# LuoGroup2023/PanTax

Measured on AMD Instinct MI355X. Metric: PAO wall-time (s) + Mreads/s: packed reads + DB (graphs and their unique-trio index) resident in HBM -> abundance tables; the metric's own GAF -> abundance quantity is value_gaf_to_tables (files -> tables, never `value`), higher is better.
Workload: dtype int64+f64

## Files before the change

pantax_amd/csrc/api_step.cpp:

```cpp
#include <algorithm>
#include <cmath>
#include <chrono>
#include <cstdio>
#include <cstdlib>
#include <cstring>
#include <vector>
#include "lad.hpp"

using namespace ptx;

namespace {
struct SpOut { Db *db; uint8_t *keep; double *absolute; int slot; };
void copy_species_out(void *arg) {
    SpOut *o = static_cast<SpOut *>(arg);
    const uint32_t S = o->db->S;
    std::memcpy(o->absolute, o->db->h_sp_out[o->slot].p, sizeof(double) * S);
    std::memcpy(o->keep, o->db->h_sp_out[o->slot].p + sizeof(double) * S, S);
}

int step_enqueue(pantax_hip_ctx *ctx, pantax_hip_db *db, pantax_hip_reads *reads, const double *avg_len, const pantax_hip_step_config *cfg) {
    if (db->d_node_rec.p == nullptr) return fail(ctx, PANTAX_HIP_E_STATE, "profile_step: the db was uploaded without graphs (ranges only)");
    if (db->step_inflight >= 2) return fail(ctx, PANTAX_HIP_E_STATE, "profile_step_enqueue: two steps of this db are already in flight; collect one first");
    const uint32_t S = db->S;
    const int slot = db->step_enq;
    const auto t_begin = std::chrono::steady_clock::now();
    double marks[8] = {0}; int n_marks = 0;
    auto mark = [&]() { if (n_marks < 8) marks[n_marks++] = std::chrono::duration<double, std::milli>(std::chrono::steady_clock::now() - t_begin).count(); };
    struct SlowReport { double *m; int *n; bool on; ~SlowReport() {
        if (*n && m[*n - 1] > 2.0 && on) {
            std::fprintf(stderr, "[step_enqueue] slow call, ms at marks (trio enqueued, bin+species, prezero+cov prepare, coverage, strain):");
            for (int i = 0; i < *n; ++i) std::fprintf(stderr, " %.2f", m[i]);
            std::fprintf(stderr, "\n");
        } } } slow_report{marks, &n_marks, ctx->cfg.trace};
    bool forked = false;
    if (cfg->rebuild_trio && !(db->trio_prefetched && db->trio_built)) { db->trio_built = false; db->cov_done = false; db->U = 0; }
    db->trio_prefetched = false;
    if (!db->trio_built) {
        if (db->trio_free_valid && !ctx->cfg.trio_after_step) PTX_HIP(ctx, hipStreamWaitEvent(ctx->stream2, db->ev_trio_free, 0));
        else {
            PTX_HIP(ctx, hipEventRecord(ctx->ev_seq, ctx->stream));
            PTX_HIP(ctx, hipStreamWaitEvent(ctx->stream2, ctx->ev_seq, 0));
        }
        hipStream_t main_stream = ctx->stream;
        ctx->stream_main = main_stream; ctx->stream = ctx->stream2;
        const int rc = trio_index_build(ctx, db, false);
        const hipError_t e = hipEventRecord(ctx->ev_fork, ctx->stream2);
        ctx->stream = main_stream; ctx->stream_main = nullptr;
        if (rc != 0) return rc;
        PTX_HIP(ctx, e);
        forked = true;
    }
    struct ForkGuard {
        Ctx *c; Db *d; bool armed;
        ~ForkGuard() { if (armed) { (void)hipStreamSynchronize(c->stream2); d->trio_built = false; d->cov_done = false; } }
    } fork_guard{ctx, db, forked};
// ... 98 lines not shown
```

pantax_amd/csrc/common.hpp:

```cpp
#pragma once
#include <hip/hip_runtime.h>
#include <cstdint>
#include <cstdio>
#include <map>
#include <functional>
#include <mutex>
#include <cstring>
#include <atomic>
#include <string>
#include <vector>
#include "../../include/pantax_hip.h"

#ifndef TRIO_LH_PACK
#define TRIO_LH_PACK 0
#endif
namespace ptx {

struct Ctx;
#if TRIO_LH_PACK
using trio_len_t = uint2;
#else
using trio_len_t = uint32_t;
#endif

// ... 86 lines not shown
    int stage_ch_mb = 0;
    bool stream_prio = true;
    int dev_cache_gb = -1;
    bool numa_bind = true;
    uint64_t gaf_piece_bytes = 0;
    int db_groups = 0;
    uint64_t db_path_steps_max = 0;
    std::string trio_path;
    std::string trio_rows;
    int uniq_hash = -1;
    std::string mask;
    std::string row_sort;
    std::string objective;
    std::string read_strain_route, evidence_route, depth_route, near_miss_route, hap_pairs_route;
    int hap_pairs_chunk = 0;
    int depth_grid = 0;
    int near_miss_words = 0;
    bool cov_general = false;
    std::string cov_long;
    int covl_shape = -1;
    bool cov_count = false;
    int cov_clean_async = -1;
    bool cov_self_clean = false;
    bool walk_sum_in_bin = false;
    int ncs_prefix_min = 48;
    bool ncs_no_prefix = false;
    bool cov_arena_verify = false;
    int cov_item_groups = 0;
    int tv_u = 4, tv_rounds = 4, tf_u = 8, tf_rounds = 1, rows_u = 1, tb_slots = 256, trio_xcd = 3, cov_shape = -1, covf_shape = -1, cov_xcd = 0, group_bucket_bits = 0;
    uint32_t tv_ablate = 0, cov_ablate = 0, ssn_ablate = 0;
    bool trio_two_pass = false;
    std::string bin_route;
    std::string node_pass;
    std::string lad_shape;
    std::string scan_tile;
    std::string ssn_keys;
    bool ssn_poison_keys = false;
    int ssn_ties_async = -1;
    bool no_absent_skip = false;
    bool ssn_debug = false, scan_no_huge = false, flag_rank_chained = false, ratio_kernel = false, mask_pass = false, trio_free_at_filter = false,
         trio_after_step = false;
};
int ctx_set_option(CtxConfig &cfg, const char *name, const char *value);

struct NumaInfo {
    int node = -1;
    std::vector<int> cpus;
};

struct Ctx {
    std::recursive_mutex mu;
    CtxConfig cfg;
    NumaInfo numa;
    int device = 0;
    hipStream_t stream = nullptr;
    hipStream_t stream_main = nullptr;
    hipStream_t stream2 = nullptr;
    hipStream_t stream_up = nullptr;
    hipEvent_t ev_fork = nullptr;
    hipEvent_t ev_ssn_fork = nullptr, ev_ssn_join = nullptr;
    hipEvent_t ev_seq = nullptr;
    std::string err;
    std::mutex err_mu;
    bool timing = false;
    std::string timing_filter;
    std::vector<TimedLaunch> pending;
// ... 423 lines not shown
```

pantax_amd/csrc/ctx.cpp:

```cpp
#include <exception>
#include <cstdarg>
#include <algorithm>
#include <atomic>
#include <cstring>
#include <functional>
#include <chrono>
#include <condition_variable>
#include <cstdio>
#include <mutex>
#include <thread>
#include <unistd.h>
#include <fcntl.h>
#include <sched.h>
#include <pthread.h>
#include <sys/syscall.h>
#include <fstream>
#include <cctype>
#include <cstddef>
#include <cstdlib>
#include "common.hpp"
#include "lad.hpp"

namespace ptx {

// ... 39 lines not shown
KTimer::~KTimer() {
    if (!start) return;
    (void)hipEventRecord(stop, ctx->stream);
    ctx->pending.push_back({name, start, stop});
}

int collect_timings(Ctx *ctx) {
    if (ctx->pending.empty()) return 0;
    PTX_HIP(ctx, hipStreamSynchronize(ctx->stream));
    for (auto &t : ctx->pending) {
        float ms = 0.f;
        if (hipEventElapsedTime(&ms, t.start, t.stop) == hipSuccess) {
            auto &a = ctx->acc[t.name];
            a.first += 1;
            a.second += ms;
        }
        ctx->free_events.push_back({t.start, t.stop});
    }
    ctx->pending.clear();
    return 0;
}

namespace {
enum OptKind { O_BOOL, O_INT, O_U32, O_U64, O_STR };
struct OptDesc { const char *name; OptKind kind; size_t off; };
#define OPT(nm, kind, field) {nm, kind, offsetof(CtxConfig, field)}
const OptDesc OPTIONS[] = {
    OPT("hip_trace", O_BOOL, trace), OPT("stage_threads", O_INT, stage_threads), OPT("stage_ch_mb", O_INT, stage_ch_mb), OPT("stream_prio", O_BOOL, stream_prio), OPT("numa_bind", O_BOOL, numa_bind), OPT("dev_cache_gb", O_INT, dev_cache_gb),
    OPT("gaf_piece_bytes", O_U64, gaf_piece_bytes), OPT("db_path_steps_max", O_U64, db_path_steps_max), OPT("db_groups", O_INT, db_groups), OPT("trio_path", O_STR, trio_path), OPT("trio_rows", O_STR, trio_rows), OPT("trio_two_pass", O_BOOL, trio_two_pass), OPT("uniq_hash", O_INT, uniq_hash),
    OPT("mask", O_STR, mask), OPT("row_sort", O_STR, row_sort), OPT("objective", O_STR, objective), OPT("read_strain_route", O_STR, read_strain_route), OPT("evidence_route", O_STR, evidence_route), OPT("depth_route", O_STR, depth_route), OPT("depth_grid", O_INT, depth_grid), OPT("near_miss_route", O_STR, near_miss_route), OPT("near_miss_words", O_INT, near_miss_words), OPT("hap_pairs_route", O_STR, hap_pairs_route), OPT("hap_pairs_chunk", O_INT, hap_pairs_chunk),
    OPT("cov_general", O_BOOL, cov_general), OPT("cov_long", O_STR, cov_long), OPT("covl_shape", O_INT, covl_shape), OPT("cov_count", O_BOOL, cov_count), OPT("cov_self_clean", O_BOOL, cov_self_clean), OPT("cov_clean_async", O_INT, cov_clean_async), OPT("cov_arena_verify", O_BOOL, cov_arena_verify), OPT("ncs_no_prefix", O_BOOL, ncs_no_prefix), OPT("ncs_prefix_min", O_INT, ncs_prefix_min), OPT("walk_sum_in_bin", O_BOOL, walk_sum_in_bin), OPT("cov_item_groups", O_INT, cov_item_groups), OPT("tv_u", O_INT, tv_u), OPT("tv_rounds", O_INT, tv_rounds), OPT("tf_u", O_INT, tf_u), OPT("tf_rounds", O_INT, tf_rounds),
    OPT("rows_u", O_INT, rows_u), OPT("tb_slots", O_INT, tb_slots), OPT("trio_xcd", O_INT, trio_xcd), OPT("cov_shape", O_INT, cov_shape),
    OPT("covf_shape", O_INT, covf_shape), OPT("cov_xcd", O_INT, cov_xcd), OPT("group_bucket_bits", O_INT, group_bucket_bits), OPT("tv_ablate", O_U32, tv_ablate),
    OPT("cov_ablate", O_U32, cov_ablate), OPT("ssn_ablate", O_U32, ssn_ablate), OPT("no_absent_skip", O_BOOL, no_absent_skip), OPT("node_pass", O_STR, node_pass), OPT("bin_route", O_STR, bin_route), OPT("lad_shape", O_STR, lad_shape), OPT("ssn_debug", O_BOOL, ssn_debug),
    OPT("ssn_keys", O_STR, ssn_keys), OPT("ssn_poison_keys", O_BOOL, ssn_poison_keys), OPT("ssn_ties_async", O_INT, ssn_ties_async),
    OPT("scan_no_huge", O_BOOL, scan_no_huge), OPT("scan_tile", O_STR, scan_tile), OPT("flag_rank_chained", O_BOOL, flag_rank_chained), OPT("ratio_kernel", O_BOOL, ratio_kernel),
    OPT("mask_pass", O_BOOL, mask_pass), OPT("trio_free_at_filter", O_BOOL, trio_free_at_filter), OPT("trio_after_step", O_BOOL, trio_after_step),
};
#undef OPT
}

int ctx_set_option(CtxConfig &cfg, const char *name, const char *value) {
    if (!name) return PANTAX_HIP_E_INVALID;
    static const CtxConfig defaults;
    for (const OptDesc &o : OPTIONS) {
        if (std::strcmp(o.name, name) != 0) continue;
        char *dst = reinterpret_cast<char *>(&cfg) + o.off;
        const char *def = reinterpret_cast<const char *>(&defaults) + o.off;
        char *end = nullptr;
        switch (o.kind) {
        case O_BOOL: *reinterpret_cast<bool *>(dst) = value ? !(value[0] == '0' || value[0] == '\0' || value[0] == 'n' || value[0] == 'f') : *reinterpret_cast<const bool *>(def); return 0;
        case O_INT: { if (!value) { *reinterpret_cast<int *>(dst) = *reinterpret_cast<const int *>(def); return 0; }
                      const long v = std::strtol(value, &end, 10); if (end == value) return PANTAX_HIP_E_INVALID; *reinterpret_cast<int *>(dst) = (int)v; return 0; }
        case O_U32: { if (!value) { *reinterpret_cast<uint32_t *>(dst) = *reinterpret_cast<const uint32_t *>(def); return 0; }
                      const unsigned long long v = std::strtoull(value, &end, 10); if (end == value) return PANTAX_HIP_E_INVALID; *reinterpret_cast<uint32_t *>(dst) = (uint32_t)v; return 0; }
        case O_U64: { if (!value) { *reinterpret_cast<uint64_t *>(dst) = *reinterpret_cast<const uint64_t *>(def); return 0; }
                      const unsigned long long v = std::strtoull(value, &end, 10); if (end == value) return PANTAX_HIP_E_INVALID; *reinterpret_cast<uint64_t *>(dst) = (uint64_t)v; return 0; }
        case O_STR: *reinterpret_cast<std::string *>(dst) = value ? value : ""; return 0;
        }
    }
    return PANTAX_HIP_E_INVALID;
}

static void config_from_env(CtxConfig &cfg) {
    for (const OptDesc &o : OPTIONS) {
        std::string env = "PANTAX_";
        for (const char *p = o.name; *p; ++p) env += (char)std::toupper((unsigned char)*p);
// ... 591 lines not shown
```

pantax_amd/csrc/sample_sort_nodes.hip:

```cpp
#include <algorithm>
#include <cstdio>
#include <vector>
#include "ssn_device.hpp"

namespace ptx {

size_t sample_sort_nodes_ws_elems(uint32_t S, uint64_t seg_bound, uint64_t V) { return ssn_plan(S, seg_bound, V).total_words; }

int sample_sort_nodes(Ctx *ctx, const double *ab, const uint64_t *mask, const uint32_t *d_node_base, uint32_t S, uint64_t seg_bound, uint64_t V,
                      uint64_t *rows16, uint64_t *const k[3], int pack_shift, uint32_t *d_ws, uint32_t *d_n, const RowPatterns *pat,
                      const RowMaskSource *haps, const NodeCovSource *fused) {
    if (S == 0 || V == 0) {
        PTX_HIP(ctx, hipMemsetAsync(d_n, 0, sizeof(uint32_t), ctx->stream));
        if (pat) { PTX_HIP(ctx, hipMemsetAsync(pat->d_K, 0, sizeof(uint32_t), ctx->stream)); PTX_HIP(ctx, hipMemsetAsync(pat->sp_pat_off, 0, (S + 1) * sizeof(uint32_t), ctx->stream));
                   PTX_HIP(ctx, hipMemsetAsync(pat->pat_start, 0, sizeof(uint32_t), ctx->stream)); }
        return 0;
    }
    if (seg_bound > SSN_MAX_SEG) return fail(ctx, PANTAX_HIP_E_LIMIT, "sample_sort_nodes: a segment of %llu nodes exceeds %llu", (unsigned long long)seg_bound, (unsigned long long)SSN_MAX_SEG);
    if (S > 65535) return fail(ctx, PANTAX_HIP_E_LIMIT, "sample_sort_nodes: %u segments exceed the launch grid", S);
    if (haps) { if (haps->max_haps > 64) return fail(ctx, PANTAX_HIP_E_INVALID, "sample_sort_nodes: masks from haplotype words take species of at most 64 haplotypes"); }
    else if (!mask) return fail(ctx, PANTAX_HIP_E_INVALID, "sample_sort_nodes: neither a mask array nor haplotype words");
    if (fused && (!haps || !fused->bases || !fused->bit_off || !fused->full || !fused->bitmap || !fused->amax || !fused->nvalid || !fused->nzsum || !fused->nzcnt))
        return fail(ctx, PANTAX_HIP_E_INVALID, "sample_sort_nodes: the fused node pass takes haplotype words and the coverage arena");
    if (!fused && !ab) return fail(ctx, PANTAX_HIP_E_INVALID, "sample_sort_nodes: no abundance array");

    const int keys_all = ssn_keys_all(ctx->cfg.ssn_keys.c_str(), pat != nullptr);
    if (keys_all < 0) return fail(ctx, PANTAX_HIP_E_INVALID, "sample_sort_nodes: option ssn_keys=%s%s", ctx->cfg.ssn_keys.c_str(), pat ? "" : " (a sort whose caller reads the keys stores all of them)");

    const SsnPlan pl = ssn_plan(S, seg_bound, V);
    Sn sn;
    sn.node_base = d_node_base; sn.ab = ab; sn.mask = haps ? nullptr : mask;
    if (haps) sn.hp = *haps;
    if (fused) { sn.fz = *fused; sn.ab = nullptr; sn.hp.cov = nullptr; }
    sn.G = pl.G; sn.per = pl.per;
    sn.ablate = ctx->cfg.ssn_ablate;
    sn.skip_empty = ctx->cfg.no_absent_skip ? 0u : 1u;
    sn.ws = d_ws + pl.ws;
    sn.cntm = d_ws + pl.cntm;
    sn.stage_cnt = d_ws + pl.stage_cnt;
    sn.c0p = reinterpret_cast<double *>(d_ws + pl.c0p);
    sn.c0 = pat ? pat->c0 : nullptr;
    sn.seg_n = d_ws + pl.seg_n; sn.seg_out = d_ws + pl.seg_out;
    uint32_t *sub_k = d_ws + pl.sub_k;
    sn.ids = reinterpret_cast<uint16_t *>(d_ws + pl.ids);
    sn.npart = reinterpret_cast<NodePartial *>(d_ws + pl.npart);
    sn.rows = reinterpret_cast<ulonglong2 *>(rows16);
    sn.stage = reinterpret_cast<ulonglong2 *>(rows16) + V;
    sn.ksp = pack_shift >= 0 ? nullptr : k[0];
    sn.km = pack_shift >= 0 ? k[0] : k[1];
    sn.ka = pack_shift >= 0 ? k[1] : k[2];
    sn.pack_shift = pack_shift;
    sn.keys_all = (uint32_t)keys_all;
    if (!keys_all && ctx->cfg.ssn_poison_keys) {
        PTX_TRY(byte_fill(ctx, sn.km, 0xA5, V * sizeof(uint64_t)));
        if (sn.ksp) PTX_TRY(byte_fill(ctx, sn.ksp, 0xA5, V * sizeof(uint64_t)));
    }

    { KTimer t(ctx, "ssn_sample_kernel");
      ssn_sample_launch(ctx, sn, S, fused != nullptr); }
    if (fused) {
        KTimer t(ctx, "node_rows_kernel");
        ssn_node_rows_launch(ctx, sn, S, haps->max_haps);
    } else {
        KTimer t(ctx, "ssn_hist_kernel");
        ssn_hist_launch(ctx, sn, S, haps != nullptr, haps ? haps->max_haps : 0u);
    }
    { KTimer t(ctx, "ssn_offsets_kernel");
      ssn_offsets_launch(ctx, sn, S, d_n); }
    const bool clocked = ctx->timing && ctx->timing_filter.empty();
    const bool ties_async = ssn_ties_async(ctx->cfg.ssn_ties_async, clocked, ctx->stream_main != nullptr, ctx->stream2 != nullptr);
    struct TieJoin {
        Ctx *c; bool armed;
        ~TieJoin() { if (armed) (void)hipStreamSynchronize(c->stream2); }
    } tie_join{ctx, false};
    if (ties_async) {
        if (!ctx->ev_ssn_fork) PTX_HIP(ctx, hipEventCreateWithFlags(&ctx->ev_ssn_fork, hipEventDisableTiming));
        if (!ctx->ev_ssn_join) PTX_HIP(ctx, hipEventCreateWithFlags(&ctx->ev_ssn_join, hipEventDisableTiming));
        PTX_HIP(ctx, hipEventRecord(ctx->ev_ssn_fork, ctx->stream));
        PTX_HIP(ctx, hipStreamWaitEvent(ctx->stream2, ctx->ev_ssn_fork, 0));
        hipStream_t main_stream = ctx->stream;
        ctx->stream_main = main_stream; ctx->stream = ctx->stream2;
        tie_join.armed = true;
        { KTimer t(ctx, "ssn_ties_kernel");
          ssn_ties_launch(ctx, sn, S, pl.tie_grid); }
        const hipError_t e = hipEventRecord(ctx->ev_ssn_join, ctx->stream2);
        ctx->stream = main_stream; ctx->stream_main = nullptr;
        PTX_HIP(ctx, e);
    }
    { KTimer t(ctx, "ssn_scatter_kernel");
      ssn_scatter_launch(ctx, sn, S); }
    if (!ties_async) {
        KTimer t(ctx, "ssn_ties_kernel");
        ssn_ties_launch(ctx, sn, S, pl.tie_grid);
    }
    { KTimer t(ctx, "ssn_local_wave_kernel");
// ... 38 lines not shown
```

pantax_amd/csrc/ssn_device.hpp:

```cpp
#pragma once
#include "primitives.hpp"
#include "wave.hpp"
#include "ssn_plan.hpp"

namespace ptx {

constexpr int SN_NSPLIT = SN_NLEAF - 1;
constexpr int SN_CAP = 4096;
constexpr int SN_WAVE_CAP = 512;
constexpr int SN_WAVE_CAP2 = 1024;
constexpr uint16_t SN_NO_ROW = 0xFFFFu;
static_assert(sizeof(NodePartial) == 4 * SN_NODE_PARTIAL_WORDS && alignof(NodePartial) == 8, "ssn_plan lays out [S x G] NodePartial at an even word offset");

struct Key2 { uint64_t m, a; };
__device__ __forceinline__ bool less2(const Key2 &x, const Key2 &y) { return (x.m < y.m) | ((x.m == y.m) & (x.a < y.a)); }
__device__ __forceinline__ bool eq2(const Key2 &x, const Key2 &y) { return (x.m == y.m) & (x.a == y.a); }

struct Sn {
    const uint32_t *node_base;
    const double *ab;
    const uint64_t *mask;
    RowMaskSource hp;
    NodeCovSource fz;
    NodePartial *npart;
// ... 92 lines not shown
__device__ __forceinline__ bool sn_pair_mixed(const ulonglong2 *__restrict__ tree, uint32_t j, uint64_t *mv = nullptr) {
    if (j == 0 || j >= (uint32_t)SN_NSPLIT) { if (mv) *mv = 0; return true; }
    const uint64_t ma = tree[tree_node(j - 1)].x, mb = tree[tree_node(j)].x;
    if (mv) *mv = mb;
    return ma != mb;
}

__device__ __forceinline__ void sn_tiles(const Sn &sn, uint32_t n, uint32_t g, uint32_t &t0, uint32_t &t1) {
    const uint32_t nt = (n + SN_TILE - 1) / SN_TILE;
    t0 = g * sn.per; t1 = t0 + sn.per;
    if (t0 > nt) t0 = nt;
    if (t1 > nt) t1 = nt;
}

template <int NT>
__device__ __forceinline__ void bitonic2(uint64_t *km, uint64_t *ka, uint32_t N) {
    for (uint32_t k = 2; k <= N; k <<= 1)
        for (uint32_t j = k >> 1; j > 0; j >>= 1) {
            for (uint32_t t = threadIdx.x; t < N / 2; t += NT) {
                const uint32_t i = ((t & ~(j - 1)) << 1) | (t & (j - 1)), l = i | j;
                const Key2 x{km[i], ka[i]}, y{km[l], ka[l]};
                const bool up = (i & k) == 0;
                if (up ? less2(y, x) : less2(x, y)) { km[i] = y.m; ka[i] = y.a; km[l] = x.m; ka[l] = x.a; }
            }
            __syncthreads();
        }
}

#ifdef SSN_ABLATE
#define SSN_ABL(b) ((sn.ablate & (b)) != 0u)
#else
#define SSN_ABL(b) false
#endif

void ssn_sample_launch(Ctx *ctx, const Sn &sn, uint32_t S, bool fused);
void ssn_node_rows_launch(Ctx *ctx, const Sn &sn, uint32_t S, uint32_t max_haps);
void ssn_hist_launch(Ctx *ctx, const Sn &sn, uint32_t S, bool haps, uint32_t max_haps);
void ssn_offsets_launch(Ctx *ctx, const Sn &sn, uint32_t S, uint32_t *d_n);
void ssn_scatter_launch(Ctx *ctx, const Sn &sn, uint32_t S);
void ssn_ties_launch(Ctx *ctx, const Sn &sn, uint32_t S, uint32_t tie_grid);
void ssn_local_launch(Ctx *ctx, const Sn &sn, uint32_t S);
void ssn_patterns_launch(Ctx *ctx, const Sn &sn, uint32_t S, uint32_t *sub_k, const RowPatterns &pat, const uint32_t *d_n);

}
```

pantax_amd/csrc/ssn_node_pass.hip:

```cpp
#include "ssn_device.hpp"

namespace ptx {

namespace {
template <bool HAPS>
__global__ void __launch_bounds__(256) ssn_hist_kernel(Sn sn) {
    __shared__ ulonglong2 tree[SN_NLEAF];
    __shared__ uint32_t s_hist[SN_NBUCKET];
    extern __shared__ unsigned long long s_dyn_tab[];
    __shared__ int s_bit[64];
    __shared__ unsigned long long s_acc[2 * 64];
    const uint32_t s = blockIdx.y, g = blockIdx.x, o = sn.node_base[s], n = sn.node_base[s + 1] - o;
    uint32_t *w = sn.w(s);
    if (n == 0 || w[SN_OFF_FLAGS] != 0) return;
    if (HAPS && sn.skip_empty && sn.hp.sp_p[s] <= 0) {
        uint32_t *row0 = sn.cntm + ((size_t)s * sn.G + g) * SN_NBUCKET;
        for (int i = threadIdx.x; i < SN_NBUCKET; i += 256) row0[i] = 0u;
        if (threadIdx.x == 0) { sn.stage_cnt[(size_t)s * sn.G + g] = 0u; if (sn.c0) sn.c0p[(size_t)s * sn.G + g] = 0.0; }
        return;
    }
    uint32_t t0, t1;
    sn_tiles(sn, n, g, t0, t1);
    const ulonglong2 *gt = reinterpret_cast<const ulonglong2 *>(w + SN_OFF_TREE);
    __shared__ uint32_t s_nstage;
// ... 92 lines not shown
                }
            }
        }
    }
    __syncthreads();
    uint32_t *row = sn.cntm + ((size_t)s * sn.G + g) * SN_NBUCKET;
    for (int i = threadIdx.x; i < SN_NBUCKET; i += 256) row[i] = s_hist[i];
    if (threadIdx.x == 0) sn.stage_cnt[(size_t)s * sn.G + g] = s_nstage;
    if (sn.c0) {
        __shared__ double s_c[4];
        cacc = wave_reduce(cacc, [](double x, double y) { return x + y; });
        if (lane == 0) s_c[threadIdx.x >> 6] = cacc;
        __syncthreads();
        if (threadIdx.x == 0) sn.c0p[(size_t)s * sn.G + g] = (s_c[0] + s_c[1]) + (s_c[2] + s_c[3]);
    }
    if (HAPS && p0 > 0 && sn.hp.ratio) {
#pragma unroll
        for (int k = 0; k < 8; ++k) {
            if (k >= p0) break;
            const unsigned long long cs = wave_reduce(c8[k], [](unsigned long long x, unsigned long long y) { return x + y; });
            const unsigned long long ls = wave_reduce(l8[k], [](unsigned long long x, unsigned long long y) { return x + y; });
            if (lane == 0) {
                if (cs) atomicAdd(&s_acc[2 * k], cs);
                if (ls) atomicAdd(&s_acc[2 * k + 1], ls);
            }
        }
        __syncthreads();
        if ((int)threadIdx.x < 2 * p0 && s_acc[threadIdx.x]) atomicAdd(&sn.hp.ratio[2 * h0 + threadIdx.x], s_acc[threadIdx.x]);
    }
}

constexpr int SN_HALF = SN_ITEMS >= 8 ? SN_ITEMS / 2 : SN_ITEMS;
static_assert(SN_ITEMS % SN_HALF == 0, "whole halves");
__global__ void __launch_bounds__(256) node_rows_kernel(Sn sn) {
    __shared__ ulonglong2 tree[SN_NLEAF];
    __shared__ uint32_t s_hist[SN_NBUCKET];
    extern __shared__ unsigned long long s_dyn_tab[];
    __shared__ int s_bit[64];
    __shared__ unsigned long long s_acc[2 * 64];
    const uint32_t s = blockIdx.y, g = blockIdx.x, o = sn.node_base[s], n = sn.node_base[s + 1] - o;
    uint32_t *w = sn.w(s);
    if (n == 0 || w[SN_OFF_FLAGS] != 0) return;
    uint32_t t0, t1;
    sn_tiles(sn, n, g, t0, t1);
    if (sn.skip_empty && sn.hp.sp_p[s] <= 0) {
        uint32_t *row0 = sn.cntm + ((size_t)s * sn.G + g) * SN_NBUCKET;
        for (int i = threadIdx.x; i < SN_NBUCKET; i += 256) row0[i] = 0u;
        if (threadIdx.x == 0) { sn.stage_cnt[(size_t)s * sn.G + g] = 0u; if (sn.c0) sn.c0p[(size_t)s * sn.G + g] = 0.0; }
        if (!sn.fz.active || sn.fz.active[s]) {
            NodeAcc acc;
            for (uint32_t t = t0; t < t1; ++t)
#pragma unroll
                for (int r = 0; r < SN_ITEMS; ++r) {
                    const uint32_t i = t * SN_TILE + (uint32_t)r * 256u + threadIdx.x;
                    if (i < n) acc.add((double)(long long)sn.fz.bases[o + i] / (double)sn.hp.node_len[o + i], sn.fz.min_depth);
                }
            sn_block_partial<4>(acc, sn.npart + (size_t)s * sn.G + g);
        }
        return;
    }
    const ulonglong2 *gt = reinterpret_cast<const ulonglong2 *>(w + SN_OFF_TREE);
    __shared__ uint32_t s_nstage;
    for (int i = threadIdx.x; i < SN_NBUCKET; i += 256) s_hist[i] = 0;
    if (threadIdx.x == 0) s_nstage = 0;
    if (t0 < t1) for (int i = threadIdx.x; i < SN_NLEAF; i += 256) tree[i] = gt[i];
    const uint64_t h0 = sn.hp.hap_off[s], nh = sn.hp.hap_off[s + 1] - h0;
    int p0 = sn.hp.sp_p[s];
    if (p0 <= 0 || p0 > 64 || nh > 64) p0 = 0;
    const int nbyte = p0 ? (int)((nh + 7) / 8) : 0;
    if (threadIdx.x < 64) s_bit[threadIdx.x] = (p0 && threadIdx.x < nh) ? sn.hp.hap_bit[h0 + threadIdx.x] : -1;
    if (threadIdx.x < 128) s_acc[threadIdx.x] = 0;
    __syncthreads();
    for (int b = 0; b < nbyte; ++b) {
        unsigned long long e = 0ull;
#pragma unroll
        for (int i = 0; i < 8; ++i) { const int bit = s_bit[8 * b + i]; if (((threadIdx.x >> i) & 1u) && bit >= 0) e |= 1ull << bit; }
        s_dyn_tab[b * 256 + threadIdx.x] = e;
    }
    __syncthreads();
    unsigned long long c8[8] = {0, 0, 0, 0, 0, 0, 0, 0}, l8[8] = {0, 0, 0, 0, 0, 0, 0, 0};
    const uint32_t stage0 = o + t0 * SN_TILE;
    const int lane = threadIdx.x & 63;
    const uint32_t wave64 = (uint32_t)__builtin_amdgcn_readfirstlane((int)(threadIdx.x >> 6)) << 6;
    double cacc = 0.0;
    NodeAcc nacc;
    constexpr int HALF = SN_HALF;
    for (uint32_t t = t0; t < t1; ++t) {
#pragma unroll
      for (int hb = 0; hb < SN_ITEMS; hb += HALF) {
        const uint32_t base = t * SN_TILE + (uint32_t)hb * 256u + threadIdx.x;
        double av[HALF];
        uint64_t mv[HALF];
        uint32_t cv[HALF], lv[HALF];
        {
            unsigned long long bs[HALF];
            uint32_t fw[HALF];
            uint64_t g0[HALF];
#pragma unroll
            for (int r = 0; r < HALF; ++r) {
                const uint32_t i = base + (uint32_t)r * 256u;
                const bool in = i < n;
                lv[r] = in ? sn.hp.node_len[o + i] : 0u;
                bs[r] = in ? sn.fz.bases[o + i] : 0ull;
                fw[r] = in ? sn.fz.full[(o + i) >> 5] : 0u;
                mv[r] = in ? sn.hp.node_haps[o + i] : 0ull;
            }
#pragma unroll
            for (int r = 0; r < HALF; ++r) {
                const uint32_t i0 = t * SN_TILE + (uint32_t)(hb + r) * 256u + wave64;
                g0[r] = i0 < n ? sn.fz.bit_off[o + i0] : 0ull;
            }
#pragma unroll
            for (int r = 0; r < HALF; ++r) g0[r] += wave_incl_scan_dpp(lv[r]) - lv[r];
            bool whole[HALF];
#pragma unroll
            for (int r = 0; r < HALF; ++r) {
                const unsigned long long hm = mv[r];
                unsigned long long m = 0ull;
                for (int b = 0; b < nbyte; ++b) m |= s_dyn_tab[b * 256 + (int)((hm >> (8 * b)) & 255ull)];
                mv[r] = m;
                whole[r] = (fw[r] >> ((o + base + (uint32_t)r * 256u) & 31u)) & 1u;
            }
            uint32_t bw0[HALF], bw1[HALF];
#pragma unroll
            for (int r = 0; r < HALF; ++r) {
                const bool count = lv[r] != 0u && mv[r] != 0ull && !whole[r];
                bw0[r] = count ? sn.fz.bitmap[g0[r] >> 5] : 0u;
                bw1[r] = count ? sn.fz.bitmap[(g0[r] + lv[r] - 1) >> 5] : 0u;
            }
#pragma unroll
            for (int r = 0; r < HALF; ++r) {
                const uint32_t i = base + (uint32_t)r * 256u;
                uint32_t c = whole[r] ? lv[r] : 0u;
                if (lv[r] != 0u && mv[r] != 0ull && !whole[r]) {
                    const uint64_t g1 = g0[r] + lv[r], w0 = g0[r] >> 5, w1 = (g1 - 1) >> 5;
                    const uint32_t m0 = 0xFFFFFFFFu << (g0[r] & 31), m1 = 0xFFFFFFFFu >> (31 - (uint32_t)((g1 - 1) & 31));
                    c = w0 == w1 ? __popc(bw0[r] & m0 & m1) : __popc(bw0[r] & m0) + __popc(bw1[r] & m1);
                    for (uint64_t ww = w0 + 1; ww < w1; ++ww) c += __popc(sn.fz.bitmap[ww]);
                }
                cv[r] = c;
                av[r] = 0.0;
                if (i < n) {
                    av[r] = (double)(long long)bs[r] / (double)lv[r];
                    nacc.add(av[r], sn.fz.min_depth);
                }
            }
        }
#pragma unroll
        for (int r = 0; r < HALF; ++r) {
            {
                const unsigned long long m = mv[r];
                if (m) {
                    const unsigned long long c = cv[r], l = lv[r];
#pragma unroll
                    for (int k = 0; k < 8; ++k)
                        if (k < p0) { const bool on = (m >> k) & 1ull; c8[k] += on ? c : 0ull; l8[k] += on ? l : 0ull; }
                    unsigned long long rest = m >> 8;
                    while (rest) {
                        const int k = __ffsll((long long)rest) - 1 + 8;
                        rest &= rest - 1;
                        if (c) atomicAdd(&s_acc[2 * k], c);
                        atomicAdd(&s_acc[2 * k + 1], l);
                    }
                }
            }
            uint32_t id = SN_NO_ROW;
            const uint64_t abits = (uint64_t)__double_as_longlong(av[r]);
            if (av[r] > 0.0 && mv[r] == 0ull) cacc += av[r];
            if (av[r] > 0.0 && mv[r] != 0ull) {
                const Key2 key{mv[r], abits};
                uint32_t k = 1;
#pragma unroll
                for (int l = 0; l < SN_LEVELS; ++l) { const ulonglong2 nd = tree[k]; k = 2u * k + (less2(Key2{nd.x, nd.y}, key) ? 1u : 0u); }
                const uint32_t lo = k - (uint32_t)SN_NLEAF;
                uint32_t eq = 0;
                if (lo < (uint32_t)SN_NSPLIT) { const ulonglong2 nd = tree[tree_node(lo)]; eq = eq2(Key2{nd.x, nd.y}, key) ? 1u : 0u; }
                id = 2u * lo + eq;
                atomicAdd(&s_hist[id], 1u);
            }
            const bool travels = id != SN_NO_ROW && !(id & 1u);
            const unsigned long long bal = __ballot(travels);
            if (bal) {
                uint32_t wbase = 0;
                if (lane == 0) wbase = atomicAdd(&s_nstage, (uint32_t)__popcll(bal));
                wbase = (uint32_t)__builtin_amdgcn_readfirstlane((int)wbase);
                if (travels) {
                    const uint32_t pos = stage0 + wbase + (uint32_t)__popcll(bal & ((1ull << lane) - 1ull));
                    sn.stage[pos] = make_ulonglong2(mv[r], abits);
                    sn.ids[pos] = (uint16_t)id;
                }
            }
        }
      }
    }
    __syncthreads();
    sn_block_partial<4>(nacc, sn.npart + (size_t)s * sn.G + g);
    uint32_t *row = sn.cntm + ((size_t)s * sn.G + g) * SN_NBUCKET;
    for (int i = threadIdx.x; i < SN_NBUCKET; i += 256) row[i] = s_hist[i];
    if (threadIdx.x == 0) sn.stage_cnt[(size_t)s * sn.G + g] = s_nstage;
    if (sn.c0) {
        __shared__ double s_c[4];
        cacc = wave_reduce(cacc, [](double x, double y) { return x + y; });
        if (lane == 0) s_c[threadIdx.x >> 6] = cacc;
        __syncthreads();
        if (threadIdx.x == 0) sn.c0p[(size_t)s * sn.G + g] = (s_c[0] + s_c[1]) + (s_c[2] + s_c[3]);
    }
    if (p0 > 0 && sn.hp.ratio) {
#pragma unroll
        for (int k = 0; k < 8; ++k) {
            if (k >= p0) break;
            const unsigned long long cs = wave_reduce(c8[k], [](unsigned long long x, unsigned long long y) { return x + y; });
            const unsigned long long ls = wave_reduce(l8[k], [](unsigned long long x, unsigned long long y) { return x + y; });
            if (lane == 0) {
                if (cs) atomicAdd(&s_acc[2 * k], cs);
                if (ls) atomicAdd(&s_acc[2 * k + 1], ls);
            }
        }
        __syncthreads();
        if ((int)threadIdx.x < 2 * p0 && s_acc[threadIdx.x]) atomicAdd(&sn.hp.ratio[2 * h0 + threadIdx.x], s_acc[threadIdx.x]);
    }
}

__global__ void __launch_bounds__(64) node_rows_final_kernel(Sn sn) {
    const uint32_t s = blockIdx.x, n = sn.node_base[s + 1] - sn.node_base[s];
    double mx = -INFINITY, zs = 0.0; unsigned long long nv = 0, zc = 0;
    if (n != 0 && sn.fz.active && !sn.fz.active[s]) mx = 0.0;
    else if (n != 0) {
        const uint32_t nt = (n + SN_TILE - 1) / SN_TILE, ng = n <= (uint32_t)SN_SAMPLE ? 1u : (nt + sn.per - 1) / sn.per;
        for (uint32_t g = threadIdx.x; g < ng; g += 64) { const NodePartial p = sn.npart[(size_t)s * sn.G + g]; mx = fmax(mx, p.mx); zs += p.zs; nv += p.nv; zc += p.zc; }
    }
    mx = wave_reduce(mx, [](double x, double y) { return fmax(x, y); });
    zs = wave_reduce(zs, [](double x, double y) { return x + y; });
    nv = wave_reduce(nv, [](unsigned long long x, unsigned long long y) { return x + y; });
    zc = wave_reduce(zc, [](unsigned long long x, unsigned long long y) { return x + y; });
    if (threadIdx.x == 0) { sn.fz.amax[s] = mx; sn.fz.nvalid[s] = (uint32_t)nv; sn.fz.nzsum[s] = zs; sn.fz.nzcnt[s] = (uint32_t)zc; }
}
}

void ssn_node_rows_launch(Ctx *ctx, const Sn &sn, uint32_t S, uint32_t max_haps) {
    hipLaunchKernelGGL(node_rows_kernel, dim3(sn.G, S), dim3(256), (size_t)((max_haps + 7) / 8) * 256 * sizeof(unsigned long long), ctx->stream, sn);
    hipLaunchKernelGGL(node_rows_final_kernel, dim3(S), dim3(64), 0, ctx->stream, sn);
}

void ssn_hist_launch(Ctx *ctx, const Sn &sn, uint32_t S, bool haps, uint32_t max_haps) {
    if (haps) hipLaunchKernelGGL(ssn_hist_kernel<true>, dim3(sn.G, S), dim3(256), (size_t)((max_haps + 7) / 8) * 256 * sizeof(unsigned long long), ctx->stream, sn);
    else hipLaunchKernelGGL(ssn_hist_kernel<false>, dim3(sn.G, S), dim3(256), 0, ctx->stream, sn);
}

}
```

pantax_amd/csrc/ssn_plan.cpp:

```cpp
#include "ssn_plan.hpp"
#include <algorithm>
#include <cstring>

namespace ptx {

SsnPlan ssn_plan(uint32_t S, uint64_t seg_bound, uint64_t V) {
    SsnPlan p;
    const uint64_t nt = std::max<uint64_t>(1, (seg_bound + SN_TILE - 1) / SN_TILE);
    const uint64_t target = SN_TARGET_WGS;
    uint64_t per = (nt * S + target - 1) / target;
    if (per < 1) per = 1;
    if (per > nt) per = nt;
    p.per = (uint32_t)per;
    p.G = (uint32_t)((nt + per - 1) / per);
    p.tie_grid = (uint32_t)((seg_bound + SN_TIE_ROWS - 1) / SN_TIE_ROWS);

    const size_t SG = (size_t)S * p.G;
    size_t at = 0;
    auto take = [&at](size_t words, bool even = false) {
        if (even) at += at & 1u;
        const size_t off = at;
        at += words;
        return off;
    };
    p.ws = take((size_t)S * SN_WS_WORDS);
    p.cntm = take(SG * SN_NBUCKET);
    p.stage_cnt = take(SG);
    p.c0p = take(2 * SG, true);
    p.seg_n = take(S);
    p.seg_out = take((size_t)S + 1);
    p.sub_k = take((size_t)SN_NWH * S);
    p.ids = take((size_t)((V + 1) / 2));
    p.npart = take(SN_NODE_PARTIAL_WORDS * SG, true);
    p.total_words = at;
    return p;
}

int ssn_keys_all(const char *option, bool has_patterns) {
    if (!option || !*option || std::strcmp(option, "auto") == 0) return has_patterns ? 0 : 1;
    if (std::strcmp(option, "all") == 0) return 1;
    if (std::strcmp(option, "needed") == 0) return has_patterns ? 0 : -1;
    return -1;
}

bool ssn_ties_async(int option, bool clocked, bool on_side_stream, bool have_side_stream) {
    if (clocked || on_side_stream || !have_side_stream) return false;
    return option > 0 || (option < 0 && SSN_TIES_ASYNC_AUTO);
}

}
```

pantax_amd/csrc/ssn_plan.hpp:

```cpp
#pragma once
#include <cstddef>
#include <cstdint>

namespace ptx {

#ifndef SN_LEVELS
#define SN_LEVELS 10
#endif
constexpr int SN_SAMPLE = 4096;
constexpr int SN_NLEAF = 1 << SN_LEVELS;
constexpr int SN_NBUCKET = 2 * SN_NLEAF;
#ifndef SN_ITEMS_N
#define SN_ITEMS_N 8
#endif
constexpr int SN_ITEMS = SN_ITEMS_N;
constexpr int SN_TILE = 256 * SN_ITEMS;
constexpr uint32_t SN_TARGET_WGS = 8192;
constexpr uint32_t SN_TIE_ROWS = 8192;
#ifndef SN_HEAD_PAIRS
#define SN_HEAD_PAIRS 64
#endif
constexpr int SN_HP = SN_HEAD_PAIRS, SN_NWH = SN_NLEAF / SN_HP;
constexpr bool SSN_TIES_ASYNC_AUTO = false;
constexpr uint64_t SSN_MAX_SEG = 1ull << 26;

constexpr size_t SN_OFF_FLAGS = 0;
constexpr size_t SN_OFF_TREE = 4;
constexpr size_t SN_OFF_SAMP = SN_OFF_TREE + 4 * SN_NLEAF;
constexpr size_t SN_OFF_START = SN_OFF_SAMP + 2 * 2 * SN_SAMPLE;
constexpr size_t SN_OFF_MED = SN_OFF_START + SN_NBUCKET + 4;
constexpr size_t SN_OFF_BIG = SN_OFF_MED + SN_NBUCKET;
constexpr size_t SN_WS_WORDS = SN_OFF_BIG + SN_NBUCKET;
static_assert(SN_WS_WORDS % 4 == 0, "16-byte tree nodes");

constexpr size_t SN_NODE_PARTIAL_WORDS = 8;

struct SsnPlan {
    uint32_t G = 1, per = 1;
    uint32_t tie_grid = 1;
    size_t ws = 0;
    size_t cntm = 0;
    size_t stage_cnt = 0;
    size_t c0p = 0;
    size_t seg_n = 0;
    size_t seg_out = 0;
    size_t sub_k = 0;
    size_t ids = 0;
    size_t npart = 0;
    size_t total_words = 0;
};
SsnPlan ssn_plan(uint32_t S, uint64_t seg_bound, uint64_t V);

int ssn_keys_all(const char *option, bool has_patterns);
bool ssn_ties_async(int option, bool clocked, bool on_side_stream, bool have_side_stream);

}
```

pantax_amd/csrc/wave.hpp:

```cpp
#pragma once
#include <hip/hip_runtime.h>
#include <cstdint>

namespace ptx {

template <int CTRL>
__device__ __forceinline__ uint32_t dpp32(uint32_t v) { return (uint32_t)__builtin_amdgcn_update_dpp((int)v, (int)v, CTRL, 0xF, 0xF, false); }
template <int CTRL, class T>
__device__ __forceinline__ T dpp(T v) {
    static_assert(sizeof(T) == 4 || sizeof(T) == 8, "32- or 64-bit lanes");
    if constexpr (sizeof(T) == 4) {
        uint32_t u; __builtin_memcpy(&u, &v, 4); u = dpp32<CTRL>(u);
        T r; __builtin_memcpy(&r, &u, 4); return r;
    } else {
        uint64_t u; __builtin_memcpy(&u, &v, 8);
        uint32_t lo = dpp32<CTRL>((uint32_t)u), hi = dpp32<CTRL>((uint32_t)(u >> 32));
        u = ((uint64_t)hi << 32) | lo;
        T r; __builtin_memcpy(&r, &u, 8); return r;
    }
}
template <class T>
__device__ __forceinline__ T lane_get(T v, int lane) {
    if constexpr (sizeof(T) == 4) {
        uint32_t u; __builtin_memcpy(&u, &v, 4); u = (uint32_t)__builtin_amdgcn_readlane((int)u, lane);
        T r; __builtin_memcpy(&r, &u, 4); return r;
    } else {
        uint64_t u; __builtin_memcpy(&u, &v, 8);
        uint32_t lo = (uint32_t)__builtin_amdgcn_readlane((int)(uint32_t)u, lane), hi = (uint32_t)__builtin_amdgcn_readlane((int)(uint32_t)(u >> 32), lane);
        u = ((uint64_t)hi << 32) | lo;
        T r; __builtin_memcpy(&r, &u, 8); return r;
    }
}
template <class T, class Op>
__device__ __forceinline__ T wave_reduce(T v, Op op) {
    v = op(v, dpp<0xB1>(v)); v = op(v, dpp<0x4E>(v)); v = op(v, dpp<0x124>(v)); v = op(v, dpp<0x128>(v));
    return op(op(lane_get(v, 0), lane_get(v, 16)), op(lane_get(v, 32), lane_get(v, 48)));
}
template <class T, class Op>
__device__ __forceinline__ T row_reduce(T v, Op op) {
    v = op(v, dpp<0xB1>(v)); v = op(v, dpp<0x4E>(v)); v = op(v, dpp<0x124>(v)); v = op(v, dpp<0x128>(v));
    return v;
}
template <class A, class B, class Better>
__device__ __forceinline__ void wave_reduce_pair(A &a, B &b, Better better) {
#define PTX_PAIR_STEP(CTRL) { A a2 = dpp<CTRL>(a); B b2 = dpp<CTRL>(b); if (better(a2, b2, a, b)) { a = a2; b = b2; } }
    PTX_PAIR_STEP(0xB1) PTX_PAIR_STEP(0x4E) PTX_PAIR_STEP(0x124) PTX_PAIR_STEP(0x128)
#undef PTX_PAIR_STEP
    A ra = lane_get(a, 0); B rb = lane_get(b, 0);
#pragma unroll
    for (int r = 16; r < 64; r += 16) { A a2 = lane_get(a, r); B b2 = lane_get(b, r); if (better(a2, b2, ra, rb)) { ra = a2; rb = b2; } }
    a = ra; b = rb;
}

__device__ __forceinline__ uint32_t wave_shr1(uint32_t v, uint32_t fill = 0u) {
    return (uint32_t)__builtin_amdgcn_update_dpp((int)fill, (int)v, 0x138, 0xF, 0xF, false);
}
__device__ __forceinline__ uint32_t wave_shr1z(uint32_t v) { return (uint32_t)__builtin_amdgcn_update_dpp(0, (int)v, 0x138, 0xF, 0xF, true); }
__device__ __forceinline__ uint32_t wave_incl_scan_dpp(uint32_t v) {
    v += (uint32_t)__builtin_amdgcn_update_dpp(0, (int)v, 0x111, 0xF, 0xF, true);
    v += (uint32_t)__builtin_amdgcn_update_dpp(0, (int)v, 0x112, 0xF, 0xF, true);
    v += (uint32_t)__builtin_amdgcn_update_dpp(0, (int)v, 0x114, 0xF, 0xF, true);
    v += (uint32_t)__builtin_amdgcn_update_dpp(0, (int)v, 0x118, 0xF, 0xF, true);
    v += (uint32_t)__builtin_amdgcn_update_dpp(0, (int)v, 0x142, 0xA, 0xF, false);
    v += (uint32_t)__builtin_amdgcn_update_dpp(0, (int)v, 0x143, 0xC, 0xF, false);
    return v;
}

__device__ __forceinline__ uint32_t wave_incl_scan(uint32_t v) {
    const int lane = threadIdx.x & 63;
#pragma unroll
    for (int d = 1; d < 64; d <<= 1) {
        uint32_t t = __shfl_up(v, d);
        if (lane >= d) v += t;
    }
    return v;
}

template <int NT>
__device__ __forceinline__ uint32_t block_excl_scan(uint32_t v, uint32_t *s_wave , uint32_t *block_total) {
    const int lane = threadIdx.x & 63, wave = threadIdx.x >> 6;
    uint32_t incl = wave_incl_scan(v);
    if (lane == 63) s_wave[wave] = incl;
    __syncthreads();
    uint32_t woff = 0, tot = 0;
#pragma unroll
    for (int w = 0; w < NT / 64; ++w) {
        uint32_t t = s_wave[w];
        if (w < wave) woff += t;
        tot += t;
// ... 9 lines not shown
```

Before: 6658.

## Load node bitmap range cooperatively per wave and count bits via popcount scan

```diff
diff --git a/pantax_amd/csrc/api_step.cpp b/pantax_amd/csrc/api_step.cpp
--- a/pantax_amd/csrc/api_step.cpp
+++ b/pantax_amd/csrc/api_step.cpp
@@ -6,6 +6,7 @@
 #include <cstring>
 #include <vector>
 #include "lad.hpp"
+#include "ssn_plan.hpp"
 
 using namespace ptx;
 
@@ -21,6 +22,8 @@
 int step_enqueue(pantax_hip_ctx *ctx, pantax_hip_db *db, pantax_hip_reads *reads, const double *avg_len, const pantax_hip_step_config *cfg) {
     if (db->d_node_rec.p == nullptr) return fail(ctx, PANTAX_HIP_E_STATE, "profile_step: the db was uploaded without graphs (ranges only)");
     if (db->step_inflight >= 2) return fail(ctx, PANTAX_HIP_E_STATE, "profile_step_enqueue: two steps of this db are already in flight; collect one first");
+    if (ssn_node_bits(ctx->cfg.node_bits.c_str(), ctx->cfg.node_bits_words) < 0)
+        return fail(ctx, PANTAX_HIP_E_INVALID, "profile_step: option node_bits is \"range\" or \"gather\" and node_bits_words 0, 1 or 2, not \"%s\" and %d", ctx->cfg.node_bits.c_str(), ctx->cfg.node_bits_words);
     const uint32_t S = db->S;
     const int slot = db->step_enq;
     const auto t_begin = std::chrono::steady_clock::now();
diff --git a/pantax_amd/csrc/common.hpp b/pantax_amd/csrc/common.hpp
--- a/pantax_amd/csrc/common.hpp
+++ b/pantax_amd/csrc/common.hpp
@@ -142,6 +142,8 @@
     bool trio_two_pass = false;
     std::string bin_route;
     std::string node_pass;
+    std::string node_bits;
+    int node_bits_words = 0;
     std::string lad_shape;
     std::string scan_tile;
     std::string ssn_keys;
diff --git a/pantax_amd/csrc/ctx.cpp b/pantax_amd/csrc/ctx.cpp
--- a/pantax_amd/csrc/ctx.cpp
+++ b/pantax_amd/csrc/ctx.cpp
@@ -95,7 +95,7 @@
     OPT("cov_general", O_BOOL, cov_general), OPT("cov_long", O_STR, cov_long), OPT("covl_shape", O_INT, covl_shape), OPT("cov_count", O_BOOL, cov_count), OPT("cov_self_clean", O_BOOL, cov_self_clean), OPT("cov_clean_async", O_INT, cov_clean_async), OPT("cov_arena_verify", O_BOOL, cov_arena_verify), OPT("ncs_no_prefix", O_BOOL, ncs_no_prefix), OPT("ncs_prefix_min", O_INT, ncs_prefix_min), OPT("walk_sum_in_bin", O_BOOL, walk_sum_in_bin), OPT("cov_item_groups", O_INT, cov_item_groups), OPT("tv_u", O_INT, tv_u), OPT("tv_rounds", O_INT, tv_rounds), OPT("tf_u", O_INT, tf_u), OPT("tf_rounds", O_INT, tf_rounds),
     OPT("rows_u", O_INT, rows_u), OPT("tb_slots", O_INT, tb_slots), OPT("trio_xcd", O_INT, trio_xcd), OPT("cov_shape", O_INT, cov_shape),
     OPT("covf_shape", O_INT, covf_shape), OPT("cov_xcd", O_INT, cov_xcd), OPT("group_bucket_bits", O_INT, group_bucket_bits), OPT("tv_ablate", O_U32, tv_ablate),
-    OPT("cov_ablate", O_U32, cov_ablate), OPT("ssn_ablate", O_U32, ssn_ablate), OPT("no_absent_skip", O_BOOL, no_absent_skip), OPT("node_pass", O_STR, node_pass), OPT("bin_route", O_STR, bin_route), OPT("lad_shape", O_STR, lad_shape), OPT("ssn_debug", O_BOOL, ssn_debug),
+    OPT("cov_ablate", O_U32, cov_ablate), OPT("ssn_ablate", O_U32, ssn_ablate), OPT("no_absent_skip", O_BOOL, no_absent_skip), OPT("node_pass", O_STR, node_pass), OPT("bin_route", O_STR, bin_route), OPT("node_bits", O_STR, node_bits), OPT("node_bits_words", O_INT, node_bits_words), OPT("lad_shape", O_STR, lad_shape), OPT("ssn_debug", O_BOOL, ssn_debug),
     OPT("ssn_keys", O_STR, ssn_keys), OPT("ssn_poison_keys", O_BOOL, ssn_poison_keys), OPT("ssn_ties_async", O_INT, ssn_ties_async),
     OPT("scan_no_huge", O_BOOL, scan_no_huge), OPT("scan_tile", O_STR, scan_tile), OPT("flag_rank_chained", O_BOOL, flag_rank_chained), OPT("ratio_kernel", O_BOOL, ratio_kernel),
     OPT("mask_pass", O_BOOL, mask_pass), OPT("trio_free_at_filter", O_BOOL, trio_free_at_filter), OPT("trio_after_step", O_BOOL, trio_after_step),
diff --git a/pantax_amd/csrc/sample_sort_nodes.hip b/pantax_amd/csrc/sample_sort_nodes.hip
--- a/pantax_amd/csrc/sample_sort_nodes.hip
+++ b/pantax_amd/csrc/sample_sort_nodes.hip
@@ -26,6 +26,8 @@
 
     const int keys_all = ssn_keys_all(ctx->cfg.ssn_keys.c_str(), pat != nullptr);
     if (keys_all < 0) return fail(ctx, PANTAX_HIP_E_INVALID, "sample_sort_nodes: option ssn_keys=%s%s", ctx->cfg.ssn_keys.c_str(), pat ? "" : " (a sort whose caller reads the keys stores all of them)");
+    const int node_bits = ssn_node_bits(ctx->cfg.node_bits.c_str(), ctx->cfg.node_bits_words);
+    if (node_bits < 0) return fail(ctx, PANTAX_HIP_E_INVALID, "sample_sort_nodes: option node_bits is \"range\" or \"gather\" and node_bits_words 0, 1 or 2, not \"%s\" and %d", ctx->cfg.node_bits.c_str(), ctx->cfg.node_bits_words);
 
     const SsnPlan pl = ssn_plan(S, seg_bound, V);
     Sn sn;
@@ -60,7 +62,7 @@
       ssn_sample_launch(ctx, sn, S, fused != nullptr); }
     if (fused) {
         KTimer t(ctx, "node_rows_kernel");
-        ssn_node_rows_launch(ctx, sn, S, haps->max_haps);
+        ssn_node_rows_launch(ctx, sn, S, haps->max_haps, node_bits);
     } else {
         KTimer t(ctx, "ssn_hist_kernel");
         ssn_hist_launch(ctx, sn, S, haps != nullptr, haps ? haps->max_haps : 0u);
diff --git a/pantax_amd/csrc/ssn_device.hpp b/pantax_amd/csrc/ssn_device.hpp
--- a/pantax_amd/csrc/ssn_device.hpp
+++ b/pantax_amd/csrc/ssn_device.hpp
@@ -148,9 +148,14 @@
 #else
 #define SSN_ABL(b) false
 #endif
+#ifdef NODE_ROWS_ABLATE
+#define NRK_ABL(b) ((sn.ablate & (b)) != 0u)
+#else
+#define NRK_ABL(b) false
+#endif
 
 void ssn_sample_launch(Ctx *ctx, const Sn &sn, uint32_t S, bool fused);
-void ssn_node_rows_launch(Ctx *ctx, const Sn &sn, uint32_t S, uint32_t max_haps);
+void ssn_node_rows_launch(Ctx *ctx, const Sn &sn, uint32_t S, uint32_t max_haps, int node_bits);
 void ssn_hist_launch(Ctx *ctx, const Sn &sn, uint32_t S, bool haps, uint32_t max_haps);
 void ssn_offsets_launch(Ctx *ctx, const Sn &sn, uint32_t S, uint32_t *d_n);
 void ssn_scatter_launch(Ctx *ctx, const Sn &sn, uint32_t S);
diff --git a/pantax_amd/csrc/ssn_node_pass.hip b/pantax_amd/csrc/ssn_node_pass.hip
--- a/pantax_amd/csrc/ssn_node_pass.hip
+++ b/pantax_amd/csrc/ssn_node_pass.hip
@@ -148,6 +148,9 @@
 
 constexpr int SN_HALF = SN_ITEMS >= 8 ? SN_ITEMS / 2 : SN_ITEMS;
 static_assert(SN_ITEMS % SN_HALF == 0, "whole halves");
+constexpr int SN_HALVES = SN_ITEMS / SN_HALF;
+static_assert(2 * SN_HALF <= 64, "a lane per end of the half's items");
+template <int NB>
 __global__ void __launch_bounds__(256) node_rows_kernel(Sn sn) {
     __shared__ ulonglong2 tree[SN_NLEAF];
     __shared__ uint32_t s_hist[SN_NBUCKET];
@@ -177,6 +180,15 @@
     }
     const ulonglong2 *gt = reinterpret_cast<const ulonglong2 *>(w + SN_OFF_TREE);
     __shared__ uint32_t s_nstage;
+    const int lane = threadIdx.x & 63;
+    const uint32_t wave64 = (uint32_t)__builtin_amdgcn_readfirstlane((int)(threadIdx.x >> 6)) << 6;
+    constexpr int HALF = SN_HALF;
+    auto end_of = [&](uint32_t q) -> uint64_t {
+        const uint32_t i = q * (uint32_t)(HALF * 256) + (uint32_t)((lane >> 1) % HALF) * 256u + wave64 + (uint32_t)(lane & 1) * 64u;
+        return sn.fz.bit_off[o + (i < n ? i : n)];
+    };
+    uint64_t endv = 0;
+    if (NB && t0 < t1) endv = end_of(t0 * (uint32_t)SN_HALVES);
     for (int i = threadIdx.x; i < SN_NBUCKET; i += 256) s_hist[i] = 0;
     if (threadIdx.x == 0) s_nstage = 0;
     if (t0 < t1) for (int i = threadIdx.x; i < SN_NLEAF; i += 256) tree[i] = gt[i];
@@ -194,13 +206,13 @@
         s_dyn_tab[b * 256 + threadIdx.x] = e;
     }
     __syncthreads();
+    uint64_t eb[2 * HALF];
+#pragma unroll
+    for (int k = 0; k < 2 * HALF; ++k) eb[k] = NB ? lane_get(endv, k) : 0ull;
     unsigned long long c8[8] = {0, 0, 0, 0, 0, 0, 0, 0}, l8[8] = {0, 0, 0, 0, 0, 0, 0, 0};
     const uint32_t stage0 = o + t0 * SN_TILE;
-    const int lane = threadIdx.x & 63;
-    const uint32_t wave64 = (uint32_t)__builtin_amdgcn_readfirstlane((int)(threadIdx.x >> 6)) << 6;
     double cacc = 0.0;
     NodeAcc nacc;
-    constexpr int HALF = SN_HALF;
     for (uint32_t t = t0; t < t1; ++t) {
 #pragma unroll
       for (int hb = 0; hb < SN_ITEMS; hb += HALF) {
@@ -211,7 +223,28 @@
         {
             unsigned long long bs[HALF];
             uint32_t fw[HALF];
-            uint64_t g0[HALF];
+            uint64_t gb[HALF];
+            uint32_t ex[HALF];
+            uint32_t bw0[HALF], bw1[HALF];
+            bool fits[HALF];
+            uint32_t nwv[HALF], tbv[HALF];
+            if (NB) {
+#pragma unroll
+                for (int r = 0; r < HALF; ++r) {
+                    const uint64_t b0 = eb[2 * r], b1 = eb[2 * r + 1], w0 = b0 >> 5;
+                    const uint32_t nw = b1 > b0 ? (uint32_t)(((b1 - 1) >> 5) - w0) + 1u : 0u, cap = 64u * (uint32_t)NB;
+                    gb[r] = b0;
+                    nwv[r] = nw;
+                    tbv[r] = (uint32_t)(b1 - b0);
+                    fits[r] = nw <= cap && !NRK_ABL(1u);
+                    const uint32_t top = nw ? (nw < cap ? nw : cap) - 1u : 0u;
+                    const uint32_t *wp = sn.fz.bitmap + (nw ? w0 : 0ull);
+                    bw0[r] = wp[(uint32_t)lane < top ? (uint32_t)lane : top];
+                    bw1[r] = NB > 1 ? wp[(uint32_t)lane + 64u < top ? (uint32_t)lane + 64u : top] : 0u;
+                }
+                endv = end_of(t * (uint32_t)SN_HALVES + (uint32_t)(hb / HALF) + 1u);
+                __builtin_amdgcn_sched_barrier(0);
+            }
 #pragma unroll
             for (int r = 0; r < HALF; ++r) {
                 const uint32_t i = base + (uint32_t)r * 256u;
@@ -221,13 +254,20 @@
                 fw[r] = in ? sn.fz.full[(o + i) >> 5] : 0u;
                 mv[r] = in ? sn.hp.node_haps[o + i] : 0ull;
             }
-#pragma unroll
-            for (int r = 0; r < HALF; ++r) {
-                const uint32_t i0 = t * SN_TILE + (uint32_t)(hb + r) * 256u + wave64;
-                g0[r] = i0 < n ? sn.fz.bit_off[o + i0] : 0ull;
-            }
-#pragma unroll
-            for (int r = 0; r < HALF; ++r) g0[r] += wave_incl_scan_dpp(lv[r]) - lv[r];
+            if (!NB) {
+#pragma unroll
+                for (int r = 0; r < HALF; ++r) {
+                    const uint32_t i0 = t * SN_TILE + (uint32_t)(hb + r) * 256u + wave64;
+                    gb[r] = i0 < n ? sn.fz.bit_off[o + i0] : 0ull;
+                    fits[r] = false; nwv[r] = tbv[r] = 0u;
+                }
+            }
+#pragma unroll
+            for (int r = 0; r < HALF; ++r) ex[r] = wave_incl_scan_dpp(lv[r]) - lv[r];
+            if (NB) {
+#pragma unroll
+                for (int k = 0; k < 2 * HALF; ++k) eb[k] = lane_get(endv, k);
+            }
             bool whole[HALF];
 #pragma unroll
             for (int r = 0; r < HALF; ++r) {
@@ -237,20 +277,40 @@
                 mv[r] = m;
                 whole[r] = (fw[r] >> ((o + base + (uint32_t)r * 256u) & 31u)) & 1u;
             }
-            uint32_t bw0[HALF], bw1[HALF];
 #pragma unroll
             for (int r = 0; r < HALF; ++r) {
-                const bool count = lv[r] != 0u && mv[r] != 0ull && !whole[r];
-                bw0[r] = count ? sn.fz.bitmap[g0[r] >> 5] : 0u;
-                bw1[r] = count ? sn.fz.bitmap[(g0[r] + lv[r] - 1) >> 5] : 0u;
+                if (NB && fits[r]) continue;
+                const bool count = lv[r] != 0u && mv[r] != 0ull && !whole[r] && !NRK_ABL(1u);
+                const uint64_t g0 = gb[r] + ex[r];
+                bw0[r] = count ? sn.fz.bitmap[g0 >> 5] : 0u;
+                bw1[r] = count ? sn.fz.bitmap[(g0 + lv[r] - 1) >> 5] : 0u;
             }
 #pragma unroll
             for (int r = 0; r < HALF; ++r) {
                 const uint32_t i = base + (uint32_t)r * 256u;
+                const bool count = lv[r] != 0u && mv[r] != 0ull && !whole[r] && !NRK_ABL(1u);
                 uint32_t c = whole[r] ? lv[r] : 0u;
-                if (lv[r] != 0u && mv[r] != 0ull && !whole[r]) {
-                    const uint64_t g1 = g0[r] + lv[r], w0 = g0[r] >> 5, w1 = (g1 - 1) >> 5;
-                    const uint32_t m0 = 0xFFFFFFFFu << (g0[r] & 31), m1 = 0xFFFFFFFFu >> (31 - (uint32_t)((g1 - 1) & 31));
+                if (NB && fits[r]) {
+                    const uint32_t nw = nwv[r], last = nw ? nw - 1u : 0u;
+                    const uint32_t q0 = (uint32_t)lane < nw ? __popc(bw0[r]) : 0u, s0 = wave_incl_scan_dpp(q0);
+                    uint32_t q1 = 0u, s1 = 0u;
+                    if (NB > 1) { q1 = (uint32_t)lane + 64u < nw ? __popc(bw1[r]) : 0u; s1 = wave_incl_scan_dpp(q1) + lane_get(s0, 63); }
+                    const uint32_t f0 = ((uint32_t)gb[r] & 31u) + ex[r], j0 = f0 >> 5;
+                    uint32_t x = (uint32_t)__shfl((int)bw0[r], (int)(j0 & 63u)), px = (uint32_t)__shfl((int)(s0 - q0), (int)(j0 & 63u));
+                    if (NB > 1) {
+                        const uint32_t y = (uint32_t)__shfl((int)bw1[r], (int)(j0 & 63u)), py = (uint32_t)__shfl((int)(s1 - q1), (int)(j0 & 63u));
+                        if (j0 & 64u) { x = y; px = py; }
+                    }
+                    const uint32_t fe = ((uint32_t)gb[r] & 31u) + tbv[r];
+                    uint32_t wl = lane_get(bw0[r], (int)(last & 63u)), sl = lane_get(s0, (int)(last & 63u));
+                    if (NB > 1 && last >= 64u) { wl = lane_get(bw1[r], (int)(last & 63u)); sl = lane_get(s1, (int)(last & 63u)); }
+                    const uint32_t ce = sl - (uint32_t)__popc(wl & ~(0xFFFFFFFFu >> (31u - ((fe - 1u) & 31u))));
+                    const uint32_t e = j0 >= nw ? ce : px + (uint32_t)__popc(x & ((1u << (f0 & 31u)) - 1u));
+                    const uint32_t cc = wave_shl1(e, ce) - e;
+                    if (count) c = cc;
+                } else if (count) {
+                    const uint64_t g0 = gb[r] + ex[r], g1 = g0 + lv[r], w0 = g0 >> 5, w1 = (g1 - 1) >> 5;
+                    const uint32_t m0 = 0xFFFFFFFFu << (g0 & 31), m1 = 0xFFFFFFFFu >> (31 - (uint32_t)((g1 - 1) & 31));
                     c = w0 == w1 ? __popc(bw0[r] & m0 & m1) : __popc(bw0[r] & m0) + __popc(bw1[r] & m1);
                     for (uint64_t ww = w0 + 1; ww < w1; ++ww) c += __popc(sn.fz.bitmap[ww]);
                 }
@@ -286,11 +346,13 @@
             if (av[r] > 0.0 && mv[r] != 0ull) {
                 const Key2 key{mv[r], abits};
                 uint32_t k = 1;
+                if (NRK_ABL(2u)) k = (uint32_t)SN_NLEAF + ((uint32_t)(abits >> 30) & (uint32_t)(SN_NLEAF - 1));
+                else
 #pragma unroll
                 for (int l = 0; l < SN_LEVELS; ++l) { const ulonglong2 nd = tree[k]; k = 2u * k + (less2(Key2{nd.x, nd.y}, key) ? 1u : 0u); }
                 const uint32_t lo = k - (uint32_t)SN_NLEAF;
                 uint32_t eq = 0;
-                if (lo < (uint32_t)SN_NSPLIT) { const ulonglong2 nd = tree[tree_node(lo)]; eq = eq2(Key2{nd.x, nd.y}, key) ? 1u : 0u; }
+                if (lo < (uint32_t)SN_NSPLIT && !NRK_ABL(2u)) { const ulonglong2 nd = tree[tree_node(lo)]; eq = eq2(Key2{nd.x, nd.y}, key) ? 1u : 0u; }
                 id = 2u * lo + eq;
                 atomicAdd(&s_hist[id], 1u);
             }
@@ -353,8 +415,11 @@
 }
 }
 
-void ssn_node_rows_launch(Ctx *ctx, const Sn &sn, uint32_t S, uint32_t max_haps) {
-    hipLaunchKernelGGL(node_rows_kernel, dim3(sn.G, S), dim3(256), (size_t)((max_haps + 7) / 8) * 256 * sizeof(unsigned long long), ctx->stream, sn);
+void ssn_node_rows_launch(Ctx *ctx, const Sn &sn, uint32_t S, uint32_t max_haps, int node_bits) {
+    const size_t lds = (size_t)((max_haps + 7) / 8) * 256 * sizeof(unsigned long long);
+    if (node_bits == 0) hipLaunchKernelGGL(node_rows_kernel<0>, dim3(sn.G, S), dim3(256), lds, ctx->stream, sn);
+    else if (node_bits == 1) hipLaunchKernelGGL(node_rows_kernel<1>, dim3(sn.G, S), dim3(256), lds, ctx->stream, sn);
+    else hipLaunchKernelGGL(node_rows_kernel<2>, dim3(sn.G, S), dim3(256), lds, ctx->stream, sn);
     hipLaunchKernelGGL(node_rows_final_kernel, dim3(S), dim3(64), 0, ctx->stream, sn);
 }
 
diff --git a/pantax_amd/csrc/ssn_plan.cpp b/pantax_amd/csrc/ssn_plan.cpp
--- a/pantax_amd/csrc/ssn_plan.cpp
+++ b/pantax_amd/csrc/ssn_plan.cpp
@@ -43,6 +43,13 @@
     return -1;
 }
 
+int ssn_node_bits(const char *option, int words) {
+    if (words < 0 || words > 2) return -1;
+    if (!option || !*option || std::strcmp(option, "range") == 0) return words ? words : SSN_NODE_BITS_WORDS;
+    if (std::strcmp(option, "gather") == 0) return 0;
+    return -1;
+}
+
 bool ssn_ties_async(int option, bool clocked, bool on_side_stream, bool have_side_stream) {
     if (clocked || on_side_stream || !have_side_stream) return false;
     return option > 0 || (option < 0 && SSN_TIES_ASYNC_AUTO);
diff --git a/pantax_amd/csrc/ssn_plan.hpp b/pantax_amd/csrc/ssn_plan.hpp
--- a/pantax_amd/csrc/ssn_plan.hpp
+++ b/pantax_amd/csrc/ssn_plan.hpp
@@ -52,6 +52,8 @@
 SsnPlan ssn_plan(uint32_t S, uint64_t seg_bound, uint64_t V);
 
 int ssn_keys_all(const char *option, bool has_patterns);
+constexpr int SSN_NODE_BITS_WORDS = 2;
+int ssn_node_bits(const char *option, int words);
 bool ssn_ties_async(int option, bool clocked, bool on_side_stream, bool have_side_stream);
 
 }
diff --git a/pantax_amd/csrc/wave.hpp b/pantax_amd/csrc/wave.hpp
--- a/pantax_amd/csrc/wave.hpp
+++ b/pantax_amd/csrc/wave.hpp
@@ -55,6 +55,9 @@
 __device__ __forceinline__ uint32_t wave_shr1(uint32_t v, uint32_t fill = 0u) {
     return (uint32_t)__builtin_amdgcn_update_dpp((int)fill, (int)v, 0x138, 0xF, 0xF, false);
 }
+__device__ __forceinline__ uint32_t wave_shl1(uint32_t v, uint32_t fill = 0u) {
+    return (uint32_t)__builtin_amdgcn_update_dpp((int)fill, (int)v, 0x130, 0xF, 0xF, false);
+}
 __device__ __forceinline__ uint32_t wave_shr1z(uint32_t v) { return (uint32_t)__builtin_amdgcn_update_dpp(0, (int)v, 0x138, 0xF, 0xF, true); }
 __device__ __forceinline__ uint32_t wave_incl_scan_dpp(uint32_t v) {
     v += (uint32_t)__builtin_amdgcn_update_dpp(0, (int)v, 0x111, 0xF, 0xF, true);
```

Measured after the change: 6907, median of 6. +3.7%, better.
